# fal-ai-community/video-diffusion-speedrun

Hardware: AMD Instinct MI355X
Metric: train-step samples/sec (video latents) (higher is better)
Workload: dtype bf16; 1 GPU; C3b DiT-XL/2 bf16, latents [16,16,64,64] pt=2 -> 8192+16 tokens, ctx [512,4096]; per_gpu_batch=12, global_batch=12, parallelism=single, launch=eager, deterministic=False

## Files before the change

### video_diffusion_speedrun_amd/csrc/attention.hip

```cpp
#include "common.h"
#include <type_traits>
#include "prof.h"
#include "config.h"
#include "../../include/vds.h"
#include <cstdlib>

namespace {

constexpr float LOG2E = 1.4426950408889634f;
constexpr float LN2 = 0.6931471805599453f;

struct AttnP {
  int B, H, Lq, Lk, hd;
  const bf16_t* q; long q_sb, q_sh, q_sl;
  const bf16_t* k; long k_sb, k_sh, k_sl;
  const bf16_t* v; long v_sb, v_sh, v_sl;
  bf16_t* o; long o_sb, o_sh, o_sl;
  float* lse;
  const bf16_t* d_o; long do_sb, do_sh, do_sl;
  bf16_t* dq; long dq_sb, dq_sh, dq_sl;
  bf16_t* dk; long dk_sb, dk_sh, dk_sl;
  bf16_t* dv; long dv_sb, dv_sh, dv_sl;
  float* delta;
  float scale;
// ... 791 lines not shown
  DmaStage<64, HDP> dq_, dd_;
  dq_.init(p.q_sl, hd_q, wave, lane);
  dd_.init(p.do_sl, p.hd, wave, lane);
  const unsigned q_step = (unsigned)(64 * p.q_sl * 2), do_step = (unsigned)(64 * p.do_sl * 2);
  auto issue_tile = [&](int j, int par) {
    char* nb = qbuf + par * 2 * Q_TILE;
    dq_.issue(rq, nb, (unsigned)j * q_step, wave);
    dd_.issue(rdo, nb + Q_TILE, (unsigned)j * do_step, wave);
    if (wave == 0) {
      char* st = stats + par * 512;
      const unsigned sa = lds_addr_of(st);
      lds_dma4(rl2, sa, (unsigned)((j * 64 + lane) * 4));
      lds_dma4(rdl, sa + 256, (unsigned)((j * 64 + lane) * 4));
    }
  };
  const int nqt_all = (p.Lq + 63) / 64, jper = (nqt_all + p.q_split - 1) / (p.q_split > 0 ? p.q_split : 1);
  const int j0 = sp * jper, j1 = min(nqt_all, j0 + jper);
  issue_tile(j0, 0);

  bf16x8 kf[KSQ], vf[KSQ];
#pragma unroll
  for (int ks = 0; ks < KSQ; ++ks) {
    const int e = ks * 16 + 8 * h;
    unsigned offk = (unsigned)(((long)krow * p.k_sl + e) * 2);
    unsigned offv = (unsigned)(((long)krow * p.v_sl + e) * 2);
    if (e >= p.hd) { offk = 0xfffffff0u; offv = 0xfffffff0u; }
    kf[ks] = __builtin_bit_cast(bf16x8, __builtin_amdgcn_raw_buffer_load_b128(rk, offk, 0, 0));
    vf[ks] = __builtin_bit_cast(bf16x8, __builtin_amdgcn_raw_buffer_load_b128(rv, offv, 0, 0));
  }
  if constexpr (ONES) {
#pragma unroll
    for (int ks = 0; ks < KSQ; ++ks) kf[ks] = scale_frag(kf[ks], c);
    if (h == 1) {
      kf[KSQ - 1][0] = (__bf16)1.0f;
      kf[KSQ - 1][1] = (__bf16)1.0f;
    }
  }

  f32x16 dk[NDB], dv[NDB];
#pragma unroll
  for (int i = 0; i < NDB; ++i) { dk[i] = zero16(); dv[i] = zero16(); }
#pragma unroll
  for (int ks = 0; ks < KSQ; ++ks) { retire(kf[ks]); retire(vf[ks]); }
  VDS_WAIT_VM(0);
  __syncthreads();

  auto q_tile = [&](int j, auto PAR) {
    constexpr int par = decltype(PAR)::value;
    if (j + 1 < j1) issue_tile(j + 1, par ^ 1);
    const char* qt = qbuf + par * 2 * Q_TILE;
    const char* dot = qt + Q_TILE;
    const float* stl = reinterpret_cast<const float*>(stats + par * 512);
#pragma unroll
    for (int qb = 0; qb < 2; ++qb) {
      f32x16 s = zero16(), dp;
#pragma unroll
      for (int rg = 0; rg < 4; ++rg) {
        const f32x4 d4 = *reinterpret_cast<const f32x4*>(stl + 64 + qb * 32 + 8 * rg + 4 * h);
#pragma unroll
        for (int e = 0; e < 4; ++e) dp[4 * rg + e] = d4[e];
      }
      PRIO_HI();
#pragma unroll
      for (int ks = 0; ks < KSQ; ++ks) {
        s = mfma32(frag_row<HDP>(qt, qb * 32, ks, lane), kf[ks], s);
        dp = mfma32(frag_row<HDP>(dot, qb * 32, ks, lane), vf[ks], dp);
      }
      PRIO_LO();
      f32x16 pm;
      if constexpr (ONES) {
#pragma unroll
        for (int r = 0; r < 16; ++r) {
          const float pr = __builtin_amdgcn_exp2f(s[r]);
          pm[r] = pr;
          s[r] = pr * dp[r];
        }
      } else {
#pragma unroll
        for (int rg = 0; rg < 4; ++rg) {
          const f32x4 l4 = *reinterpret_cast<const f32x4*>(stl + qb * 32 + 8 * rg + 4 * h);
#pragma unroll
          for (int e = 0; e < 4; ++e) {
            const int r = 4 * rg + e;
            const float pr = __builtin_amdgcn_exp2f(s[r] * c - l4[e]);
            pm[r] = pr;
            s[r] = pr * dp[r];
          }
        }
      }
      PRIO_HI();
#pragma unroll
      for (int s2 = 0; s2 < 2; ++s2) {
        const bf16x8 pf = acc_frag(pm, s2);
        const bf16x8 df = acc_frag(s, s2);
#pragma unroll
        for (int db = 0; db < NDB; ++db) {
          dv[db] = mfma32(frag_tr<HDP>(dot, qb * 32 + 16 * s2, db * 32, lane), pf, dv[db]);
          dk[db] = mfma32(frag_tr<HDP>(qt, qb * 32 + 16 * s2, db * 32, lane), df, dk[db]);
        }
      }
      PRIO_LO();
    }
    VDS_WAIT_VM(0);
    __syncthreads();
  };
  for (int j = j0; j < j1; j += 2) {
    q_tile(j, std::integral_constant<int, 0>{});
    if (j + 1 < j1) q_tile(j + 1, std::integral_constant<int, 1>{});
  }
  if constexpr (KVLEN) {
    if (krow >= Lk) {
#pragma unroll
      for (int i = 0; i < NDB; ++i) { dk[i] = zero16(); dv[i] = zero16(); }
    }
  }
  if (krow < p.Lk) {
    if (p.q_split > 1) {
      float* part = p.dkv_part + ((((long)sp * p.B * p.H + bh) * p.Lk + krow) * 2) * p.hd;
      store_rows_f32<NDB>(part, dk, p.hd, h);
      store_rows_f32<NDB>(part + p.hd, dv, p.hd, h);
    } else {
      store_rows<NDB>(p.dk + b * p.dk_sb + hh * p.dk_sh + (long)krow * p.dk_sl, dk, p.scale, p.hd, h);
      store_rows<NDB>(p.dv + b * p.dv_sb + hh * p.dv_sh + (long)krow * p.dv_sl, dv, 1.0f, p.hd, h);
    }
  }
}

__device__ __forceinline__ f32x4 mfma16(bf16x8 a, bf16x8 b, f32x4 c) {
  return __builtin_amdgcn_mfma_f32_16x16x32_bf16(a, b, c, 0, 0, 0);
}
template <int HDP>
__device__ __forceinline__ bf16x8 frag16_row(const char* tile, int row0, int ks, int lane) {
  return *reinterpret_cast<const bf16x8*>(tile + imgb_off<HDP>(row0 + (lane & 15), ks * 4 + (lane >> 4)));
}
template <int HDP>
__device__ __forceinline__ bf16x8 frag16_tr(const char* tile, int r0, int d0, int lane) {
  const int g = lane >> 4, i = lane & 15, qq = i >> 2, pp = i & 3;
  const int row = r0 + 4 * g + qq;
  const int ch = (d0 >> 3) + (pp >> 1);
  const char* p0 = tile + imgb_off<HDP>(row, ch) + 8 * (pp & 1);
  const char* p1 = tile + imgb_off<HDP>(row + 16, ch) + 8 * (pp & 1);
  s16x4 lo = __builtin_amdgcn_ds_read_tr16_b64_v4i16((__attribute__((address_space(3))) s16x4*)LDS_PTR(p0));
  s16x4 hi = __builtin_amdgcn_ds_read_tr16_b64_v4i16((__attribute__((address_space(3))) s16x4*)LDS_PTR(p1));
  s16x8 r = {lo[0], lo[1], lo[2], lo[3], hi[0], hi[1], hi[2], hi[3]};
  return __builtin_bit_cast(bf16x8, r);
}
__device__ __forceinline__ bf16x8 pack2(const f32x4& a, const f32x4& b) {
  bf16x8 r;
#pragma unroll
  for (int j = 0; j < 4; ++j) { r[j] = (__bf16)a[j]; r[4 + j] = (__bf16)b[j]; }
  return r;
}

template <int HDP, bool QPAD = true, bool KVLEN = false>
__global__ __launch_bounds__(256, 2) void attn_bwd_dkv16_kernel(AttnP p) {
  static_assert(HDP == 96, "head_dim 72 layout (ones columns at 72, 73)");
  constexpr int KS = HDP / 32, NDB = 5, Q_TILE = 64 * HDP * 2;
  extern __shared__ __attribute__((aligned(16))) char smem[];
  char* qbuf = smem;
  char* stats = smem + 4 * Q_TILE;
  int bh, kt_idx;
  if (!decode_block(p.n_rt, p.tail_last, p.B * p.H, bh, kt_idx)) return;
  const int b = bh / p.H, hh = bh % p.H;
  const int tid = threadIdx.x, lane = tid & 63, g = lane >> 4;
  const int wave = __builtin_amdgcn_readfirstlane(tid >> 6);
  const int key0 = kt_idx * 128 + wave * 32;
  const int Lk = kv_len_of<KVLEN>(p, b);
  if constexpr (KVLEN) {
    if (kt_idx * 128 >= Lk) {
#pragma unroll
      for (int cb = 0; cb < 2; ++cb) {
        const int krow = key0 + cb * 16 + (lane & 15);
        store_zero_block(p.dk + b * p.dk_sb + hh * p.dk_sh + (long)krow * p.dk_sl, p.hd, g, krow < p.Lk, p.wide_dkv);
        store_zero_block(p.dv + b * p.dv_sb + hh * p.dv_sh + (long)krow * p.dv_sl, p.hd, g, krow < p.Lk, p.wide_dkv);
      }
      return;
    }
  }

  const int hd_q = QPAD ? p.hd + 8 : p.hd;
  const srd_t rq = slice_srd(p.q + b * p.q_sb + hh * p.q_sh, p.q_sl, p.Lq, hd_q);
  const srd_t rdo = slice_srd(p.d_o + b * p.do_sb + hh * p.do_sh, p.do_sl, p.Lq, p.hd);
  const __amdgpu_buffer_rsrc_t rk = slice_rsrc(p.k + b * p.k_sb + hh * p.k_sh, p.k_sl, Lk, p.hd);
  const __amdgpu_buffer_rsrc_t rv = slice_rsrc(p.v + b * p.v_sb + hh * p.v_sh, p.v_sl, Lk, p.hd);
  const long nrows = (long)p.B * p.H * p.Lq;
  const long srow0 = ((long)b * p.H + hh) * p.Lq;
  const srd_t rdl = make_srd(p.delta + srow0, (unsigned)(p.Lq * 4));
  const srd_t rl2 = make_srd(p.delta + nrows + srow0, (unsigned)(p.Lq * 4));
  const float c = p.scale * LOG2E;

  DmaStage<64, HDP, 1> dq_, dd_;
  dq_.init(p.q_sl, hd_q, wave, lane);
  dd_.init(p.do_sl, p.hd, wave, lane);
  const unsigned q_step = (unsigned)(64 * p.q_sl * 2), do_step = (unsigned)(64 * p.do_sl * 2);
  auto issue_tile = [&](int j, int par) {
    char* nb = qbuf + par * 2 * Q_TILE;
    dq_.issue(rq, nb, (unsigned)j * q_step, wave);
    dd_.issue(rdo, nb + Q_TILE, (unsigned)j * do_step, wave);
    if (wave == 0) {
      char* st = stats + par * 512;
      const unsigned sa = lds_addr_of(st);
      lds_dma4(rl2, sa, (unsigned)((j * 64 + lane) * 4));
      lds_dma4(rdl, sa + 256, (unsigned)((j * 64 + lane) * 4));
    }
  };
  issue_tile(0, 0);

  bf16x8 kf[2][KS], vf[2][KS];
#pragma unroll
  for (int cb = 0; cb < 2; ++cb) {
    const int krow = key0 + cb * 16 + (lane & 15);
#pragma unroll
    for (int ks = 0; ks < KS; ++ks) {
      const int e = ks * 32 + 8 * g;
      unsigned offk = (unsigned)(((long)krow * p.k_sl + e) * 2);
      unsigned offv = (unsigned)(((long)krow * p.v_sl + e) * 2);
      if (e >= p.hd) { offk = 0xfffffff0u; offv = 0xfffffff0u; }
      kf[cb][ks] = __builtin_bit_cast(bf16x8, __builtin_amdgcn_raw_buffer_load_b128(rk, offk, 0, 0));
      vf[cb][ks] = __builtin_bit_cast(bf16x8, __builtin_amdgcn_raw_buffer_load_b128(rv, offv, 0, 0));
    }
  }
#pragma unroll
  for (int cb = 0; cb < 2; ++cb) {
#pragma unroll
    for (int ks = 0; ks < KS; ++ks) { kf[cb][ks] = scale_frag(kf[cb][ks], c); retire(vf[cb][ks]); }
    if (g == 1) {
      kf[cb][KS - 1][0] = (__bf16)1.0f;
      kf[cb][KS - 1][1] = (__bf16)1.0f;
    }
  }

  f32x4 dk[NDB][2], dv[NDB][2];
#pragma unroll
  for (int i = 0; i < NDB; ++i)
#pragma unroll
    for (int cb = 0; cb < 2; ++cb) { dk[i][cb] = f32x4{0.f, 0.f, 0.f, 0.f}; dv[i][cb] = f32x4{0.f, 0.f, 0.f, 0.f}; }
  const int nqt = (p.Lq + 63) / 64;
  VDS_WAIT_VM(0);
  __syncthreads();

  auto q_tile = [&](int j, auto PAR, auto NKBT) {
    constexpr int par = decltype(PAR)::value;
    constexpr int NKB = decltype(NKBT)::value;
    if (j + 1 < nqt) issue_tile(j + 1, par ^ 1);
    const char* qt = qbuf + par * 2 * Q_TILE;
    const char* dot = qt + Q_TILE;
    const float* stl = reinterpret_cast<const float*>(stats + par * 512);
    if constexpr (NKB > 0)
#pragma unroll
    for (int qb = 0; qb < 2; ++qb) {
      f32x4 s[2][2], dp[2][2];
#pragma unroll
      for (int rb = 0; rb < 2; ++rb) {
        const f32x4 d4 = *reinterpret_cast<const f32x4*>(stl + 64 + qb * 32 + rb * 16 + 4 * g);
        f32x4 s0 = f32x4{0.f, 0.f, 0.f, 0.f};
        if constexpr (!QPAD) s0 = -*reinterpret_cast<const f32x4*>(stl + qb * 32 + rb * 16 + 4 * g);
#pragma unroll
        for (int cb = 0; cb < NKB; ++cb) { s[rb][cb] = s0; dp[rb][cb] = d4; }
      }
      PRIO_HI();
#pragma unroll
      for (int ks = 0; ks < KS; ++ks)
#pragma unroll
        for (int rb = 0; rb < 2; ++rb) {
          const bf16x8 aq = frag16_row<HDP>(qt, qb * 32 + rb * 16, ks, lane);
          const bf16x8 ad = frag16_row<HDP>(dot, qb * 32 + rb * 16, ks, lane);
#pragma unroll
          for (int cb = 0; cb < NKB; ++cb) {
            s[rb][cb] = mfma16(aq, kf[cb][ks], s[rb][cb]);
            dp[rb][cb] = mfma16(ad, vf[cb][ks], dp[rb][cb]);
          }
        }
      PRIO_LO();
#pragma unroll
      for (int rb = 0; rb < 2; ++rb)
#pragma unroll
        for (int cb = 0; cb < NKB; ++cb)
#pragma unroll
          for (int r = 0; r < 4; ++r) s[rb][cb][r] = __builtin_amdgcn_exp2f(s[rb][cb][r]);
#pragma unroll
      for (int rb = 0; rb < 2; ++rb)
#pragma unroll
        for (int cb = 0; cb < NKB; ++cb)
#pragma unroll
          for (int r = 0; r < 4; ++r) dp[rb][cb][r] *= s[rb][cb][r];
      bf16x8 pf[2], df[2];
#pragma unroll
      for (int cb = 0; cb < NKB; ++cb) {
        pf[cb] = pack2(s[0][cb], s[1][cb]);
        df[cb] = pack2(dp[0][cb], dp[1][cb]);
      }
      PRIO_HI();
#pragma unroll
      for (int db = 0; db < NDB; ++db) {
        const bf16x8 ado = frag16_tr<HDP>(dot, qb * 32, db * 16, lane);
        const bf16x8 aqt = frag16_tr<HDP>(qt, qb * 32, db * 16, lane);
#pragma unroll
        for (int cb = 0; cb < NKB; ++cb) {
          dv[db][cb] = mfma16(ado, pf[cb], dv[db][cb]);
          dk[db][cb] = mfma16(aqt, df[cb], dk[db][cb]);
        }
      }
      PRIO_LO();
    }
    VDS_WAIT_VM(0);
    __syncthreads();
  };
  auto run = [&](auto NKBT) {
    for (int j = 0; j < nqt; j += 2) {
      q_tile(j, std::integral_constant<int, 0>{}, NKBT);
      if (j + 1 < nqt) q_tile(j + 1, std::integral_constant<int, 1>{}, NKBT);
    }
  };
  const int nkb = min(2, max(0, (Lk - key0 + 15) >> 4));
  if (nkb == 2) run(std::integral_constant<int, 2>{});
  else if (nkb == 1) run(std::integral_constant<int, 1>{});
  else run(std::integral_constant<int, 0>{});
#pragma unroll
  for (int cb = 0; cb < 2; ++cb) {
    const int krow = key0 + cb * 16 + (lane & 15);
    float vk[NDB][4], vv[NDB][4];
#pragma unroll
    for (int db = 0; db < NDB; ++db)
#pragma unroll
      for (int e = 0; e < 4; ++e) { vk[db][e] = dk[db][cb][e]; vv[db][e] = dv[db][cb][e]; }
    if constexpr (KVLEN) {
      if (krow >= Lk) {
#pragma unroll
        for (int db = 0; db < NDB; ++db)
#pragma unroll
          for (int e = 0; e < 4; ++e) { vk[db][e] = 0.f; vv[db][e] = 0.f; }
      }
    }
    store_block_bf16_t(vk, p.scale, p.dk + b * p.dk_sb + hh * p.dk_sh + (long)krow * p.dk_sl, p.hd, g, krow < p.Lk, p.wide_dkv);
    store_block_bf16_t(vv, 1.0f, p.dv + b * p.dv_sb + hh * p.dv_sh + (long)krow * p.dv_sl, p.hd, g, krow < p.Lk, p.wide_dkv);
  }
}

__device__ __forceinline__ float max3f(float a, float b, float c) { return __builtin_fmaxf(__builtin_fmaxf(a, b), c); }
__device__ __forceinline__ float max_over_lane_groups(float x) {
  auto a = __builtin_amdgcn_permlane16_swap(__float_as_uint(x), __float_as_uint(x), false, false);
  x = fmaxf(__uint_as_float(a[0]), __uint_as_float(a[1]));
  auto b = __builtin_amdgcn_permlane32_swap(__float_as_uint(x), __float_as_uint(x), false, false);
  return fmaxf(__uint_as_float(b[0]), __uint_as_float(b[1]));
}

template <int HDP, bool KVLEN = false>
__global__ __launch_bounds__(256, 2) void attn_fwd16_kernel(AttnP p) {
  static_assert(HDP == 96, "head_dim 72 layout (ones columns at 72, 73 / 72, 76)");
  constexpr int KS = HDP / 32, NDB = 5, TILE = 64 * HDP * 2;
  extern __shared__ __attribute__((aligned(16))) char smem[];
  int bh, qt;
  if (!decode_block(p.n_rt, p.tail_last, p.B * p.H, bh, qt)) return;
  const int b = bh / p.H, hh = bh % p.H;
  const int tid = threadIdx.x, lane = tid & 63, g = lane >> 4;
  const int wave = __builtin_amdgcn_readfirstlane(tid >> 6);
  const int qrow0 = qt * 256 + wave * 64 + (lane & 15);
  const int hd_kv = p.hd + 8;
  const int Lk = kv_len_of<KVLEN>(p, b);
  if constexpr (KVLEN) {
    if (Lk == 0) {
#pragma unroll
      for (int cb = 0; cb < 4; ++cb) {
        const int qrow = qrow0 + 16 * cb;
        store_zero_block(p.o + b * p.o_sb + hh * p.o_sh + (long)qrow * p.o_sl, p.hd, g, qrow < p.Lq, p.wide_o);
        if (qrow < p.Lq && g == 0) p.lse[((long)b * p.H + hh) * p.Lq + qrow] = 0.0f;
      }
      return;
    }
  }

  const __amdgpu_buffer_rsrc_t rq = slice_rsrc(p.q + b * p.q_sb + hh * p.q_sh, p.q_sl, p.Lq, p.hd);
  const srd_t rk = slice_srd(p.k + b * p.k_sb + hh * p.k_sh, p.k_sl, Lk, hd_kv);
  const srd_t rv = slice_srd(p.v + b * p.v_sb + hh * p.v_sh, p.v_sl, Lk, hd_kv);
  DmaStage<64, HDP, 1> dk, dv;
  dk.init(p.k_sl, hd_kv, wave, lane);
  dv.init(p.v_sl, hd_kv, wave, lane);
  const unsigned k_step = (unsigned)(64 * p.k_sl * 2), v_step = (unsigned)(64 * p.v_sl * 2);
  dk.issue(rk, smem, 0, wave);
  dv.issue(rv, smem + TILE, 0, wave);

  const float c = p.scale * LOG2E;
  bf16x8 qf[4][KS];
#pragma unroll
  for (int cb = 0; cb < 4; ++cb)
#pragma unroll
    for (int ks = 0; ks < KS; ++ks) {
      const int e = ks * 32 + 8 * g;
      unsigned off = (unsigned)(((long)(qrow0 + 16 * cb) * p.q_sl + e) * 2);
      if (e >= p.hd) off = 0xfffffff0u;
      qf[cb][ks] = __builtin_bit_cast(bf16x8, __builtin_amdgcn_raw_buffer_load_b128(rq, off, 0, 0));
    }
#pragma unroll
  for (int cb = 0; cb < 4; ++cb)
#pragma unroll
    for (int ks = 0; ks < KS; ++ks) qf[cb][ks] = scale_frag(qf[cb][ks], c);

  f32x4 o[NDB][4];
#pragma unroll
  for (int db = 0; db < NDB; ++db)
#pragma unroll
    for (int cb = 0; cb < 4; ++cb) o[db][cb] = f32x4{0.f, 0.f, 0.f, 0.f};
  float m[4] = {0.f, 0.f, 0.f, 0.f};
  const int nkt = (Lk + 63) / 64;
  VDS_WAIT_VM(0);
  __syncthreads();

  auto kv_tile = [&](int j, auto PAR, auto NCBT) {
    constexpr int par = decltype(PAR)::value;
    constexpr int NCB = decltype(NCBT)::value;
    if (j + 1 < nkt) {
      char* nk = smem + (par ^ 1) * 2 * TILE;
      dk.issue(rk, nk, (unsigned)(j + 1) * k_step, wave);
      dv.issue(rv, nk + TILE, (unsigned)(j + 1) * v_step, wave);
    }
    const char* kt = smem + par * 2 * TILE;
    const char* vt = kt + TILE;
    if constexpr (NCB > 0)
#pragma unroll
    for (int kb = 0; kb < 2; ++kb) {
      f32x4 s[2][4];
#pragma unroll
      for (int rb = 0; rb < 2; ++rb)
#pragma unroll
        for (int cb = 0; cb < NCB; ++cb) s[rb][cb] = f32x4{0.f, 0.f, 0.f, 0.f};
      PRIO_HI();
#pragma unroll
      for (int ks = 0; ks < KS; ++ks)
#pragma unroll
        for (int rb = 0; rb < 2; ++rb) {
          const bf16x8 ak = frag16_row<HDP>(kt, kb * 32 + rb * 16, ks, lane);
#pragma unroll
          for (int cb = 0; cb < NCB; ++cb) s[rb][cb] = mfma16(ak, qf[cb][ks], s[rb][cb]);
        }
      PRIO_LO();
      const bool first = (j == 0) && (kb == 0);
      float mx[4];
#pragma unroll
      for (int cb = 0; cb < NCB; ++cb) {
        mx[cb] = max3f(max3f(s[0][cb][0], s[0][cb][1], s[0][cb][2]), max3f(s[0][cb][3], s[1][cb][0], s[1][cb][1]),
                       fmaxf(s[1][cb][2], s[1][cb][3]));
      }
      float mxa = mx[0];
      if constexpr (NCB == 4) mxa = fmaxf(max3f(mx[0], mx[1], mx[2]), mx[3]);
      else {
#pragma unroll
        for (int cb = 1; cb < NCB; ++cb) mxa = fmaxf(mxa, mx[cb]);
      }
      if (first || __builtin_amdgcn_ballot_w64(mxa > LAZY_THR) != 0) {
        asm volatile("; rescale" ::: "memory");
#pragma unroll
        for (int cb = 0; cb < NCB; ++cb) {
          const float mxf = max_over_lane_groups(mx[cb]);
          const float m_new = bf2f(f2bf(m[cb] + (first ? mxf : fmaxf(mxf, 0.f))));
          const float delta = m_new - m[cb];
          const float alpha = first ? 1.0f : __builtin_amdgcn_exp2f(-delta);
          m[cb] = m_new;
#pragma unroll
          for (int db = 0; db < NDB; ++db) o[db][cb] *= alpha;
#pragma unroll
          for (int rb = 0; rb < 2; ++rb)
#pragma unroll
            for (int r = 0; r < 4; ++r) s[rb][cb][r] -= delta;
          if (g == 1) qf[cb][KS - 1][0] = (__bf16)(-m_new);
        }
      }
      bf16x8 pf[4];
#pragma unroll
      for (int cb = 0; cb < NCB; ++cb) {
#pragma unroll
// ... 175 lines not shown
#pragma unroll
          for (int r = 0; r < 4; ++r) s[rb][cb][r] = __builtin_amdgcn_exp2f(s[rb][cb][r]);
#pragma unroll
      for (int rb = 0; rb < 2; ++rb)
#pragma unroll
        for (int cb = 0; cb < NCB; ++cb)
#pragma unroll
          for (int r = 0; r < 4; ++r) s[rb][cb][r] *= dp[rb][cb][r];
      bf16x8 df[NQ];
#pragma unroll
      for (int cb = 0; cb < NCB; ++cb) df[cb] = pack2(s[0][cb], s[1][cb]);
#pragma unroll
      for (int db = 0; db < NDB; ++db) {
        const bf16x8 akt = frag16_tr<HDP>(kt, kb * 32, db * 16, lane);
#pragma unroll
        for (int cb = 0; cb < NCB; ++cb) dq[db][cb] = mfma16(akt, df[cb], dq[db][cb]);
      }
    }
    VDS_WAIT_VM(0);
    __syncthreads();
  };
  auto run = [&](auto NCBT) {
    for (int j = 0; j < nkt; j += 2) {
      kv_tile(j, std::integral_constant<int, 0>{}, NCBT);
      if (j + 1 < nkt) kv_tile(j + 1, std::integral_constant<int, 1>{}, NCBT);
    }
  };
  const int ncb = min(NQ, max(0, (p.Lq - (qt * (64 * NQ) + wave * (16 * NQ)) + 15) >> 4));
  if (ncb == NQ) run(std::integral_constant<int, NQ>{});
  else if (ncb == 2) run(std::integral_constant<int, 2>{});
  else if (ncb == 1) run(std::integral_constant<int, 1>{});
  else run(std::integral_constant<int, 0>{});
#pragma unroll
  for (int cb = 0; cb < NQ; ++cb) {
    const int qrow = qrow0 + 16 * cb;
    float vq[NDB][4];
#pragma unroll
    for (int db = 0; db < NDB; ++db)
#pragma unroll
      for (int e = 0; e < 4; ++e) vq[db][e] = dq[db][cb][e];
    store_block_bf16_t(vq, p.scale, p.dq + b * p.dq_sb + hh * p.dq_sh + (long)qrow * p.dq_sl, p.hd, g, qrow < p.Lq, p.wide_dq);
  }
}

bool rows16(const void* base, long sb, long sh, long sl) {
  return base && ((uintptr_t)base % 16 == 0) && (sb % 8 == 0) && (sh % 8 == 0) && (sl % 8 == 0);
}

AttnP to_p(const vds_attn_args* a) {
  AttnP p;
  p.B = a->B; p.H = a->H; p.Lq = a->Lq; p.Lk = a->Lk; p.hd = a->head_dim;
  p.q = (const bf16_t*)a->q; p.q_sb = a->q_sb; p.q_sh = a->q_sh; p.q_sl = a->q_sl;
  p.k = (const bf16_t*)a->k; p.k_sb = a->k_sb; p.k_sh = a->k_sh; p.k_sl = a->k_sl;
  p.v = (const bf16_t*)a->v; p.v_sb = a->v_sb; p.v_sh = a->v_sh; p.v_sl = a->v_sl;
  p.o = (bf16_t*)a->o; p.o_sb = a->o_sb; p.o_sh = a->o_sh; p.o_sl = a->o_sl;
  p.lse = a->lse;
  p.d_o = (const bf16_t*)a->d_o; p.do_sb = a->do_sb; p.do_sh = a->do_sh; p.do_sl = a->do_sl;
  p.dq = (bf16_t*)a->dq; p.dq_sb = a->dq_sb; p.dq_sh = a->dq_sh; p.dq_sl = a->dq_sl;
  p.dk = (bf16_t*)a->dk; p.dk_sb = a->dk_sb; p.dk_sh = a->dk_sh; p.dk_sl = a->dk_sl;
  p.dv = (bf16_t*)a->dv; p.dv_sb = a->dv_sb; p.dv_sh = a->dv_sh; p.dv_sl = a->dv_sl;
  p.delta = a->delta;
  p.scale = 1.0f / sqrtf((float)a->head_dim);
  p.n_rt = 0;
  p.tail_last = 0;
  p.kv_pad_ones = a->kv_pad_ones;
  p.q_split = 1;
  p.dkv_part = nullptr;
  p.kv_lens = nullptr;
  const bool wide_on = vdscfg::geti(vdscfg::ATTN_WIDE_STORES) != 0;
  p.wide_o = wide_on && p.hd > 64 && rows16(p.o, p.o_sb, p.o_sh, p.o_sl);
  p.wide_dq = wide_on && p.hd > 64 && rows16(p.dq, p.dq_sb, p.dq_sh, p.dq_sl);
  p.wide_dkv = wide_on && p.hd > 64 && rows16(p.dk, p.dk_sb, p.dk_sh, p.dk_sl) && rows16(p.dv, p.dv_sb, p.dv_sh, p.dv_sl);
  return p;
}

int kernel_instance(int hd) {
  if (hd <= 0 || (hd & 7) || hd > 128) return 0;
  return hd <= 32 ? 32 : hd <= 64 ? 64 : hd <= 80 ? 80 : hd <= 96 ? 96 : 128;
}

bool strides_ok(const vds_attn_args* a, bool bwd) {
  auto ok = [](int64_t s) { return (s & 7) == 0; };
  bool r = ok(a->q_sb) && ok(a->q_sh) && ok(a->q_sl) && ok(a->k_sb) && ok(a->k_sh) && ok(a->k_sl) &&
           ok(a->v_sb) && ok(a->v_sh) && ok(a->v_sl) && (a->o_sb % 4 == 0) && (a->o_sh % 4 == 0) && (a->o_sl % 4 == 0);
  if (bwd)
    r = r && ok(a->do_sb) && ok(a->do_sh) && ok(a->do_sl) && (a->dq_sl % 4 == 0) && (a->dk_sl % 4 == 0) &&
        (a->dv_sl % 4 == 0) && (a->dq_sh % 4 == 0) && (a->dk_sh % 4 == 0) && (a->dv_sh % 4 == 0) &&
        (a->dq_sb % 4 == 0) && (a->dk_sb % 4 == 0) && (a->dv_sb % 4 == 0);
  return r;
}

constexpr int ATTN_VARIANT_DEFAULT = 7;
int attn_variant() { return vdscfg::geti(vdscfg::ATTN_MFMA16) & 7; }

template <typename K>
void set_lds(K kern, int bytes) {
  (void)hipFuncSetAttribute(reinterpret_cast<const void*>(kern), hipFuncAttributeMaxDynamicSharedMemorySize, bytes);
}

static int tail_last_for(int L, int tile) {
  return (vdscfg::geti(vdscfg::ATTN_TAIL_LAST) && L > tile && (L % tile) != 0) ? 1 : 0;
}

template <int HDP, int HDQ, bool KVLEN = false>
int run_fwd(AttnP p, hipStream_t s) {
  constexpr int LDS = 4 * 64 * HDP * 2;
  static bool once = false;
  if (!once) {
    set_lds(attn_fwd_kernel<HDP, HDQ, 2, true, KVLEN>, LDS);
    if constexpr (HDP <= 96) set_lds(attn_fwd_wide_kernel<HDP, HDQ, false, KVLEN>, LDS);
    if constexpr (HDP == 96 && HDQ == 80) set_lds(attn_fwd_wide_kernel<HDP, HDQ, true, KVLEN>, LDS);
    if constexpr (HDP == 96 && HDQ == 80) set_lds(attn_fwd16_kernel<HDP, KVLEN>, LDS);
    once = true;
  }
  const int wide = vdscfg::geti(vdscfg::ATTN_FWD_WIDE);
  bool use_wide = false;
  if constexpr (HDP == 96) use_wide = wide == 1 || (wide == 2 && p.Lq >= 2048);
  if constexpr (HDP == 64) use_wide = wide == 1 || (wide == 2 && p.Lq >= 2048);
  p.n_rt = cdiv(p.Lq, use_wide ? 256 : 128);
  p.tail_last = tail_last_for(p.Lq, use_wide ? 256 : 128);
  const int grid = cdiv(p.B * p.H, 8) * 8 * p.n_rt;
  const double fl = 4.0 * p.B * p.H * (double)p.Lq * p.Lk * p.hd;
  const bool ones_fwd = HDP == 96 && HDQ == 80 && use_wide && p.kv_pad_ones && p.hd == 72;
  vdsprof::Scope ps(ones_fwd && p.kv_pad_ones == 1 ? VDS_PROF_ATTN_FWD : VDS_PROF_ATTN_FWD_PLAIN, s, fl,
                    2.0 * p.B * p.H * p.hd * (2.0 * p.Lq + 2.0 * p.Lk));
  if constexpr (HDP == 64) {
    if (use_wide) {
      hipLaunchKernelGGL((attn_fwd_wide_kernel<HDP, HDQ, false, KVLEN>), dim3(grid), dim3(256), LDS, s, p);
      return hipGetLastError() == hipSuccess ? VDS_OK : VDS_ERR_LAUNCH;
    }
  }
  if constexpr (HDP == 96) {
    if (use_wide) {
      bool done = false;
      if constexpr (HDQ == 80) {
        if (p.kv_pad_ones && p.hd == 72) {
          if (attn_variant() & 4) hipLaunchKernelGGL((attn_fwd16_kernel<HDP, KVLEN>), dim3(grid), dim3(256), LDS, s, p);
          else hipLaunchKernelGGL((attn_fwd_wide_kernel<HDP, HDQ, true, KVLEN>), dim3(grid), dim3(256), LDS, s, p);
          done = true;
        }
      }
      if (!done) hipLaunchKernelGGL((attn_fwd_wide_kernel<HDP, HDQ, false, KVLEN>), dim3(grid), dim3(256), LDS, s, p);
      return hipGetLastError() == hipSuccess ? VDS_OK : VDS_ERR_LAUNCH;
    }
  }
  hipLaunchKernelGGL((attn_fwd_kernel<HDP, HDQ, 2, true, KVLEN>), dim3(grid), dim3(256), LDS, s, p);
  return hipGetLastError() == hipSuccess ? VDS_OK : VDS_ERR_LAUNCH;
}

int dkv_qsplit(int B, int H, int Lq, int Lk) {
  const long wgs = (long)cdiv(B * H, 8) * 8 * cdiv(Lk, 128);
  const int nqt = cdiv(Lq, 64);
  if (wgs >= 3 * 512 || nqt < 16) return 1;
  long sp = (3 * 512 + wgs - 1) / wgs;
  if (sp > nqt / 8) sp = nqt / 8;
  return (int)(sp < 1 ? 1 : sp > 16 ? 16 : sp);
}

template <int HDP, int HDQ, bool KVLEN = false>
int run_bwd(AttnP p, hipStream_t s, size_t ws_floats) {
  constexpr int LDS_DQ = 4 * 64 * HDP * 2;
  constexpr int LDS_DKV = 4 * 64 * HDP * 2 + 2 * 128 * 4;
  static bool once = false;
  if (!once) {
    set_lds(attn_bwd_dq_kernel<HDP, HDQ, false, KVLEN>, LDS_DQ);
    if constexpr (HDP == 96 && HDQ == 80) set_lds(attn_bwd_dq_kernel<HDP, HDQ, true, KVLEN>, LDS_DQ);
    set_lds(attn_bwd_dkv_kernel<HDP, HDQ, false, KVLEN>, LDS_DKV);
    if constexpr (HDP == 96 && HDQ == 80) set_lds(attn_bwd_dkv_kernel<HDP, HDQ, true>, LDS_DKV);
    if constexpr (HDP == 96 && HDQ == 80) set_lds(attn_bwd_dkv16_kernel<HDP>, LDS_DKV);
    if constexpr (HDP == 96 && HDQ == 80) set_lds(attn_bwd_dkv16_kernel<HDP, false, KVLEN>, LDS_DKV);
    if constexpr (HDP == 96 && HDQ == 80) set_lds(attn_bwd_dq16_kernel<HDP, false, KVLEN>, LDS_DQ);
    if constexpr (HDP == 96 && HDQ == 80) set_lds(attn_bwd_dq16_kernel<HDP, true, KVLEN>, LDS_DQ);
    once = true;
  }
  const long rows = (long)p.B * p.H * p.Lq;
  const double prod = 2.0 * p.B * p.H * (double)p.Lq * p.Lk * p.hd;
  const double qb = 2.0 * p.B * p.H * p.hd * (double)p.Lq, kb = 2.0 * p.B * p.H * p.hd * (double)p.Lk;
  bool fold = false;
  if constexpr (HDP == 96 && HDQ == 80) fold = p.kv_pad_ones && p.hd == 72 && (attn_variant() & 2) && vdscfg::geti(vdscfg::ATTN_DELTA_FOLD);
  auto launch_dq = [&]() {
    p.n_rt = cdiv(p.Lq, 128);
    p.tail_last = tail_last_for(p.Lq, 128);
    const int grid = cdiv(p.B * p.H, 8) * 8 * p.n_rt;
    bool ones = false;
    if constexpr (HDP == 96 && HDQ == 80) ones = p.kv_pad_ones && p.hd == 72;
    vdsprof::Scope ps(ones && p.kv_pad_ones == 1 ? VDS_PROF_ATTN_BWD_DQ : VDS_PROF_ATTN_BWD_DQ_PLAIN, s, 2.0 * prod,
                      (fold ? 4.0 : 3.0) * qb + 2.0 * kb);
    if constexpr (HDP == 96 && HDQ == 80) {
      if (fold)
        hipLaunchKernelGGL((attn_bwd_dq16_kernel<HDP, true, KVLEN>), dim3(grid), dim3(256), LDS_DQ, s, p);
      else if (ones && (attn_variant() & 2))
        hipLaunchKernelGGL((attn_bwd_dq16_kernel<HDP, false, KVLEN>), dim3(grid), dim3(256), LDS_DQ, s, p);
      else if (ones)
        hipLaunchKernelGGL((attn_bwd_dq_kernel<HDP, HDQ, true, KVLEN>), dim3(grid), dim3(256), LDS_DQ, s, p);
    }
    if (!ones) hipLaunchKernelGGL((attn_bwd_dq_kernel<HDP, HDQ, false, KVLEN>), dim3(grid), dim3(256), LDS_DQ, s, p);
  };
  if (fold) launch_dq();
  else {
    vdsprof::Scope ps(VDS_PROF_ATTN_BWD_DELTA, s, 2.0 * rows * p.hd, 2.0 * qb);
    const bool tokmajor = p.o_sh == p.hd && p.do_sh == p.hd && p.o_sl == (long)p.H * p.hd && p.do_sl == p.o_sl &&
                          (p.o_sl & 7) == 0 && (p.o_sb & 7) == 0 && (p.do_sb & 7) == 0 && p.H * p.hd <= 1536 && p.H <= 64;
    if (tokmajor)
      hipLaunchKernelGGL(attn_delta_tokmajor_kernel, dim3((unsigned)(((long)p.B * p.Lq + 3) / 4)), dim3(256), 0, s, p);
    else
      hipLaunchKernelGGL(attn_delta_kernel, dim3((unsigned)((rows + 3) / 4)), dim3(256), 0, s, p);
  }
  p.n_rt = cdiv(p.Lk, 128);
  p.tail_last = tail_last_for(p.Lk, 128);
  int grid = cdiv(p.B * p.H, 8) * 8 * p.n_rt;
  {
    bool ones_kv = false;
    if constexpr (HDP == 96 && HDQ == 80) ones_kv = p.kv_pad_ones == 1 && p.hd == 72;
    vdsprof::Scope ps(ones_kv ? VDS_PROF_ATTN_BWD_DKV : VDS_PROF_ATTN_BWD_DKV_PLAIN, s, 2.0 * prod, 2.0 * qb + 4.0 * kb);
    if constexpr (HDP == 96 && HDQ == 80) {
      if (ones_kv && (attn_variant() & 1))
        hipLaunchKernelGGL((attn_bwd_dkv16_kernel<HDP>), dim3(grid), dim3(256), LDS_DKV, s, p);
      else if (ones_kv)
        hipLaunchKernelGGL((attn_bwd_dkv_kernel<HDP, HDQ, true>), dim3(grid), dim3(256), LDS_DKV, s, p);
    }
    bool done16 = false;
    if constexpr (HDP == 96 && HDQ == 80) {
      const int x16 = vdscfg::geti(vdscfg::CROSS_DKV16);
      if (!ones_kv && p.kv_pad_ones == 2 && p.hd == 72 && x16 && ((long)grid >= 512 || x16 == 2) && (attn_variant() & 1)) {
        hipLaunchKernelGGL((attn_bwd_dkv16_kernel<HDP, false, KVLEN>), dim3(grid), dim3(256), LDS_DKV, s, p);
        done16 = true;
      }
    }
    if (!ones_kv && !done16) {
      const int force = vdscfg::geti(vdscfg::ATTN_QSPLIT);
      const int split = force > 0 ? force : dkv_qsplit(p.B, p.H, p.Lq, p.Lk);
      const size_t need = (size_t)2 * rows + (size_t)split * p.B * p.H * p.Lk * 2 * p.hd;
      if (split > 1 && (p.hd & 3) == 0 && ws_floats >= need && (p.dk_sl & 3) == 0) {
        p.q_split = split;
        p.dkv_part = p.delta + 2 * rows;
        p.tail_last = 0;
        const int g2 = cdiv(p.B * p.H, 8) * 8 * p.n_rt * split;
        hipLaunchKernelGGL((attn_bwd_dkv_kernel<HDP, HDQ, false, KVLEN>), dim3(g2), dim3(256), LDS_DKV, s, p);
        const long n = (long)p.B * p.H * p.Lk * 2 * (p.hd >> 2);
        hipLaunchKernelGGL(dkv_reduce_kernel<KVLEN>, dim3((unsigned)((n + 255) / 256)), dim3(256), 0, s, p);
        p.q_split = 1;
        p.dkv_part = nullptr;
      } else {
        hipLaunchKernelGGL((attn_bwd_dkv_kernel<HDP, HDQ, false, KVLEN>), dim3(grid), dim3(256), LDS_DKV, s, p);
      }
    }
  }
  if (!fold) launch_dq();
  return hipGetLastError() == hipSuccess ? VDS_OK : VDS_ERR_LAUNCH;
}

}

__global__ __launch_bounds__(256) void kv_pad_ones_kernel(const bf16_t* kv, long ld, int kcol0, int vcol0, bf16_t* kp,
                                                          bf16_t* vp, int B, int Lk, int H, int hd, int hdp) {
  const int cpr = hdp >> 3;
  const long n = (long)B * H * Lk * cpr;
  const long gid = (long)blockIdx.x * 256 + threadIdx.x;
  if (gid >= n) return;
  const int which = blockIdx.y;
  const int c = (int)(gid % cpr);
  const long row = gid / cpr;
  const int l = (int)(row % Lk);
  const int h = (int)((row / Lk) % H);
  const int b = (int)(row / ((long)Lk * H));
  u32x4 w = {0u, 0u, 0u, 0u};
  if (c * 8 < hd) {
    w = *reinterpret_cast<const u32x4*>(kv + ((long)b * Lk + l) * ld + (which ? vcol0 : kcol0) + h * hd + c * 8);
  } else if (c * 8 == hd) {
    w[0] = which ? 0x00003f80u : 0x3f803f80u;
    w[2] = which ? 0x00003f80u : 0u;
  }
  *reinterpret_cast<u32x4*>((which ? vp : kp) + row * hdp + c * 8) = w;
}

extern "C" int vds_kv_pad_ones(const void* kv, int64_t ld, int32_t k_col0, int32_t v_col0, void* kp, void* vp, int32_t B,
                               int32_t Lk, int32_t H, int32_t hd, int32_t hdp, vds_stream_t stream) {
  if (!kv || !kp || !vp || B <= 0 || Lk <= 0 || H <= 0 || hd <= 0) return VDS_ERR_ARG;
  if ((hd & 7) || (hdp & 7) || hdp < hd + 8 || (ld & 7) || (k_col0 & 7) || (v_col0 & 7)) return VDS_ERR_ARG;
  const long n = (long)B * H * Lk * (hdp >> 3);
  hipLaunchKernelGGL(kv_pad_ones_kernel, dim3((unsigned)((n + 255) / 256), 2), dim3(256), 0, (hipStream_t)stream,
                     (const bf16_t*)kv, (long)ld, k_col0, v_col0, (bf16_t*)kp, (bf16_t*)vp, B, Lk, H, hd, hdp);
  return hipGetLastError() == hipSuccess ? VDS_OK : VDS_ERR_LAUNCH;
}

extern "C" int vds_attn_set_variant(int32_t mask) {
  const int prev = attn_variant();
  if (mask < -1 || mask > 7) return VDS_ERR_ARG;
  vdscfg::g_val[vdscfg::ATTN_MFMA16] = mask < 0 ? ATTN_VARIANT_DEFAULT : mask;
  return prev;
}

extern "C" int vds_attn_fwd(const vds_attn_args* a, vds_stream_t stream) {
  if (!a || !a->q || !a->k || !a->v || !a->o || !a->lse || a->Lq <= 0 || a->Lk <= 0) return VDS_ERR_ARG;
  if (!strides_ok(a, false)) return VDS_ERR_ARG;
  AttnP p = to_p(a);
  hipStream_t s = (hipStream_t)stream;
  switch (kernel_instance(a->head_dim)) {
    case 32: return run_fwd<32, 32>(p, s);
    case 64: return run_fwd<64, 64>(p, s);
    case 80: return run_fwd<96, 80>(p, s);
    case 96: return run_fwd<96, 96>(p, s);
    case 128: return run_fwd<128, 128>(p, s);
    default: return VDS_ERR_UNSUPPORTED;
  }
}

extern "C" int vds_attn_fwd_kvlen(const vds_attn_args* a, const int32_t* kv_lens, vds_stream_t stream) {
  if (!a) return VDS_ERR_ARG;
  if (!kv_lens) return vds_attn_fwd(a, stream);
  if (a->kv_pad_ones == 1) return VDS_ERR_ARG;
  if (!a->q || !a->k || !a->v || !a->o || !a->lse || a->Lq <= 0 || a->Lk <= 0) return VDS_ERR_ARG;
  if (!strides_ok(a, false)) return VDS_ERR_ARG;
  AttnP p = to_p(a);
  p.kv_lens = kv_lens;
  hipStream_t s = (hipStream_t)stream;
  switch (kernel_instance(a->head_dim)) {
    case 32: return run_fwd<32, 32, true>(p, s);
    case 64: return run_fwd<64, 64, true>(p, s);
    case 80: return run_fwd<96, 80, true>(p, s);
    case 96: return run_fwd<96, 96, true>(p, s);
    case 128: return run_fwd<128, 128, true>(p, s);
    default: return VDS_ERR_UNSUPPORTED;
  }
}

extern "C" size_t vds_attn_bwd_workspace_bytes(const vds_attn_args* a) {
  if (!a || a->B <= 0 || a->H <= 0 || a->Lq <= 0) return 0;
  size_t fl = (size_t)2 * a->B * a->H * a->Lq;
  if (a->Lk > 0 && a->head_dim > 0 && a->kv_pad_ones != 1)
    fl += (size_t)dkv_qsplit(a->B, a->H, a->Lq, a->Lk) * a->B * a->H * a->Lk * 2 * a->head_dim;
  return fl * sizeof(float);
}

extern "C" int vds_attn_bwd(const vds_attn_args* a, vds_stream_t stream) {
  if (!a || !a->q || !a->k || !a->v || !a->o || !a->lse || !a->d_o || !a->dq || !a->dk || !a->dv || !a->delta)
    return VDS_ERR_ARG;
  if (!strides_ok(a, true)) return VDS_ERR_ARG;
  AttnP p = to_p(a);
  hipStream_t s = (hipStream_t)stream;
  const size_t ws = a->ws_floats > 0 ? (size_t)a->ws_floats : (size_t)2 * a->B * a->H * a->Lq;
  switch (kernel_instance(a->head_dim)) {
    case 32: return run_bwd<32, 32>(p, s, ws);
    case 64: return run_bwd<64, 64>(p, s, ws);
    case 80: return run_bwd<96, 80>(p, s, ws);
    case 96: return run_bwd<96, 96>(p, s, ws);
    case 128: return run_bwd<128, 128>(p, s, ws);
    default: return VDS_ERR_UNSUPPORTED;
  }
}

extern "C" int vds_attn_bwd_kvlen(const vds_attn_args* a, const int32_t* kv_lens, vds_stream_t stream) {
  if (!a) return VDS_ERR_ARG;
  if (!kv_lens) return vds_attn_bwd(a, stream);
  if (a->kv_pad_ones == 1) return VDS_ERR_ARG;
  if (!a->q || !a->k || !a->v || !a->o || !a->lse || !a->d_o || !a->dq || !a->dk || !a->dv || !a->delta || a->Lq <= 0 ||
      a->Lk <= 0)
    return VDS_ERR_ARG;
  if (!strides_ok(a, true)) return VDS_ERR_ARG;
  AttnP p = to_p(a);
  p.kv_lens = kv_lens;
  hipStream_t s = (hipStream_t)stream;
  const size_t ws = a->ws_floats > 0 ? (size_t)a->ws_floats : (size_t)2 * a->B * a->H * a->Lq;
  switch (kernel_instance(a->head_dim)) {
    case 32: return run_bwd<32, 32, true>(p, s, ws);
    case 64: return run_bwd<64, 64, true>(p, s, ws);
    case 80: return run_bwd<96, 80, true>(p, s, ws);
    case 96: return run_bwd<96, 96, true>(p, s, ws);
    case 128: return run_bwd<128, 128, true>(p, s, ws);
    default: return VDS_ERR_UNSUPPORTED;
  }
}
```

Baseline: 14.84 samples/s.

## Add query-split variant to dkv16 cross-attention backward kernel

```diff
diff --git a/video_diffusion_speedrun_amd/csrc/attention.hip b/video_diffusion_speedrun_amd/csrc/attention.hip
--- a/video_diffusion_speedrun_amd/csrc/attention.hip
+++ b/video_diffusion_speedrun_amd/csrc/attention.hip
@@ -967,15 +967,23 @@
   return r;
 }
 
-template <int HDP, bool QPAD = true, bool KVLEN = false>
+template <int HDP, bool QPAD = true, bool KVLEN = false, bool QSPLIT = false>
 __global__ __launch_bounds__(256, 2) void attn_bwd_dkv16_kernel(AttnP p) {
   static_assert(HDP == 96, "head_dim 72 layout (ones columns at 72, 73)");
   constexpr int KS = HDP / 32, NDB = 5, Q_TILE = 64 * HDP * 2;
   extern __shared__ __attribute__((aligned(16))) char smem[];
   char* qbuf = smem;
   char* stats = smem + 4 * Q_TILE;
-  int bh, kt_idx;
-  if (!decode_block(p.n_rt, p.tail_last, p.B * p.H, bh, kt_idx)) return;
+  int bh, kt_idx, sp = 0;
+  if constexpr (QSPLIT) {
+    const int per = p.n_rt * p.q_split, pid = blockIdx.x, idx = pid >> 3;
+    bh = (idx / per) * 8 + (pid & 7);
+    if (bh >= p.B * p.H) return;
+    kt_idx = (idx % per) % p.n_rt;
+    sp = (idx % per) / p.n_rt;
+  } else {
+    if (!decode_block(p.n_rt, p.tail_last, p.B * p.H, bh, kt_idx)) return;
+  }
   const int b = bh / p.H, hh = bh % p.H;
   const int tid = threadIdx.x, lane = tid & 63, g = lane >> 4;
   const int wave = __builtin_amdgcn_readfirstlane(tid >> 6);
@@ -983,6 +991,7 @@
   const int Lk = kv_len_of<KVLEN>(p, b);
   if constexpr (KVLEN) {
     if (kt_idx * 128 >= Lk) {
+      if constexpr (QSPLIT) return;
 #pragma unroll
       for (int cb = 0; cb < 2; ++cb) {
         const int krow = key0 + cb * 16 + (lane & 15);
@@ -1019,7 +1028,15 @@
       lds_dma4(rdl, sa + 256, (unsigned)((j * 64 + lane) * 4));
     }
   };
-  issue_tile(0, 0);
+  int js0 = 0, js1 = 0;
+  if constexpr (QSPLIT) {
+    const int n = (p.Lq + 63) / 64;
+    js0 = (int)((long)sp * n / p.q_split);
+    js1 = (int)((long)(sp + 1) * n / p.q_split);
+    if (js0 < js1) issue_tile(js0, 0);
+  } else {
+    issue_tile(0, 0);
+  }
 
   bf16x8 kf[2][KS], vf[2][KS];
 #pragma unroll
@@ -1057,7 +1074,7 @@
   auto q_tile = [&](int j, auto PAR, auto NKBT) {
     constexpr int par = decltype(PAR)::value;
     constexpr int NKB = decltype(NKBT)::value;
-    if (j + 1 < nqt) issue_tile(j + 1, par ^ 1);
+    if (j + 1 < (QSPLIT ? js1 : nqt)) issue_tile(j + 1, par ^ 1);
     const char* qt = qbuf + par * 2 * Q_TILE;
     const char* dot = qt + Q_TILE;
     const float* stl = reinterpret_cast<const float*>(stats + par * 512);
@@ -1122,15 +1139,33 @@
     __syncthreads();
   };
   auto run = [&](auto NKBT) {
-    for (int j = 0; j < nqt; j += 2) {
+    for (int j = (QSPLIT ? js0 : 0); j < (QSPLIT ? js1 : nqt); j += 2) {
       q_tile(j, std::integral_constant<int, 0>{}, NKBT);
-      if (j + 1 < nqt) q_tile(j + 1, std::integral_constant<int, 1>{}, NKBT);
+      if (j + 1 < (QSPLIT ? js1 : nqt)) q_tile(j + 1, std::integral_constant<int, 1>{}, NKBT);
     }
   };
   const int nkb = min(2, max(0, (Lk - key0 + 15) >> 4));
   if (nkb == 2) run(std::integral_constant<int, 2>{});
   else if (nkb == 1) run(std::integral_constant<int, 1>{});
   else run(std::integral_constant<int, 0>{});
+  if constexpr (QSPLIT) {
+#pragma unroll
+    for (int cb = 0; cb < 2; ++cb) {
+      const int krow = key0 + cb * 16 + (lane & 15);
+      if (krow < Lk) {
+        float* part = p.dkv_part + ((((long)sp * p.B * p.H + bh) * p.Lk + krow) * 2) * p.hd;
+#pragma unroll
+        for (int db = 0; db < NDB; ++db) {
+          const int d = db * 16 + 4 * g;
+          if (d < p.hd) {
+            *reinterpret_cast<f32x4*>(part + d) = dk[db][cb];
+            *reinterpret_cast<f32x4*>(part + p.hd + d) = dv[db][cb];
+          }
+        }
+      }
+    }
+    return;
+  }
 #pragma unroll
   for (int cb = 0; cb < 2; ++cb) {
     const int krow = key0 + cb * 16 + (lane & 15);
@@ -1612,9 +1647,11 @@
   const long wgs = (long)cdiv(B * H, 8) * 8 * cdiv(Lk, 128);
   const int nqt = cdiv(Lq, 64);
   if (wgs >= 3 * 512 || nqt < 16) return 1;
-  long sp = (3 * 512 + wgs - 1) / wgs;
-  if (sp > nqt / 8) sp = nqt / 8;
-  return (int)(sp < 1 ? 1 : sp > 16 ? 16 : sp);
+  const long cap = nqt / 8 < 16 ? nqt / 8 : 16;
+  for (long sp = 1; sp <= cap; ++sp)
+    if ((wgs * sp) % 512 == 0) return (int)sp;
+  const long sp = (3 * 512 + wgs - 1) / wgs;
+  return (int)(sp > cap ? cap : sp);
 }
 
 template <int HDP, int HDQ, bool KVLEN = false>
@@ -1629,6 +1666,7 @@
     if constexpr (HDP == 96 && HDQ == 80) set_lds(attn_bwd_dkv_kernel<HDP, HDQ, true>, LDS_DKV);
     if constexpr (HDP == 96 && HDQ == 80) set_lds(attn_bwd_dkv16_kernel<HDP>, LDS_DKV);
     if constexpr (HDP == 96 && HDQ == 80) set_lds(attn_bwd_dkv16_kernel<HDP, false, KVLEN>, LDS_DKV);
+    if constexpr (HDP == 96 && HDQ == 80) set_lds(attn_bwd_dkv16_kernel<HDP, false, KVLEN, true>, LDS_DKV);
     if constexpr (HDP == 96 && HDQ == 80) set_lds(attn_bwd_dq16_kernel<HDP, false, KVLEN>, LDS_DQ);
     if constexpr (HDP == 96 && HDQ == 80) set_lds(attn_bwd_dq16_kernel<HDP, true, KVLEN>, LDS_DQ);
     once = true;
@@ -1679,31 +1717,37 @@
       else if (ones_kv)
         hipLaunchKernelGGL((attn_bwd_dkv_kernel<HDP, HDQ, true>), dim3(grid), dim3(256), LDS_DKV, s, p);
     }
+    const int force = vdscfg::geti(vdscfg::ATTN_QSPLIT);
+    const int split = force > 0 ? force : dkv_qsplit(p.B, p.H, p.Lq, p.Lk);
+    const size_t need = (size_t)2 * rows + (size_t)split * p.B * p.H * p.Lk * 2 * p.hd;
+    const bool can_split = !ones_kv && split > 1 && (p.hd & 3) == 0 && ws_floats >= need && (p.dk_sl & 3) == 0;
+    auto launch_split = [&](auto kern) {
+      p.q_split = split;
+      p.dkv_part = p.delta + 2 * rows;
+      p.tail_last = 0;
+      const int g2 = cdiv(p.B * p.H, 8) * 8 * p.n_rt * split;
+      hipLaunchKernelGGL(kern, dim3(g2), dim3(256), LDS_DKV, s, p);
+      const long n = (long)p.B * p.H * p.Lk * 2 * (p.hd >> 2);
+      hipLaunchKernelGGL(dkv_reduce_kernel<KVLEN>, dim3((unsigned)((n + 255) / 256)), dim3(256), 0, s, p);
+      p.q_split = 1;
+      p.dkv_part = nullptr;
+    };
     bool done16 = false;
     if constexpr (HDP == 96 && HDQ == 80) {
       const int x16 = vdscfg::geti(vdscfg::CROSS_DKV16);
-      if (!ones_kv && p.kv_pad_ones == 2 && p.hd == 72 && x16 && ((long)grid >= 512 || x16 == 2) && (attn_variant() & 1)) {
-        hipLaunchKernelGGL((attn_bwd_dkv16_kernel<HDP, false, KVLEN>), dim3(grid), dim3(256), LDS_DKV, s, p);
-        done16 = true;
+      if (!ones_kv && p.kv_pad_ones == 2 && p.hd == 72 && x16 && (attn_variant() & 1)) {
+        if (can_split) {
+          launch_split(attn_bwd_dkv16_kernel<HDP, false, KVLEN, true>);
+          done16 = true;
+        } else if ((long)grid >= 512 || x16 == 2) {
+          hipLaunchKernelGGL((attn_bwd_dkv16_kernel<HDP, false, KVLEN>), dim3(grid), dim3(256), LDS_DKV, s, p);
+          done16 = true;
+        }
       }
     }
     if (!ones_kv && !done16) {
-      const int force = vdscfg::geti(vdscfg::ATTN_QSPLIT);
-      const int split = force > 0 ? force : dkv_qsplit(p.B, p.H, p.Lq, p.Lk);
-      const size_t need = (size_t)2 * rows + (size_t)split * p.B * p.H * p.Lk * 2 * p.hd;
-      if (split > 1 && (p.hd & 3) == 0 && ws_floats >= need && (p.dk_sl & 3) == 0) {
-        p.q_split = split;
-        p.dkv_part = p.delta + 2 * rows;
-        p.tail_last = 0;
-        const int g2 = cdiv(p.B * p.H, 8) * 8 * p.n_rt * split;
-        hipLaunchKernelGGL((attn_bwd_dkv_kernel<HDP, HDQ, false, KVLEN>), dim3(g2), dim3(256), LDS_DKV, s, p);
-        const long n = (long)p.B * p.H * p.Lk * 2 * (p.hd >> 2);
-        hipLaunchKernelGGL(dkv_reduce_kernel<KVLEN>, dim3((unsigned)((n + 255) / 256)), dim3(256), 0, s, p);
-        p.q_split = 1;
-        p.dkv_part = nullptr;
-      } else {
-        hipLaunchKernelGGL((attn_bwd_dkv_kernel<HDP, HDQ, false, KVLEN>), dim3(grid), dim3(256), LDS_DKV, s, p);
-      }
+      if (can_split) launch_split(attn_bwd_dkv_kernel<HDP, HDQ, false, KVLEN>);
+      else hipLaunchKernelGGL((attn_bwd_dkv_kernel<HDP, HDQ, false, KVLEN>), dim3(grid), dim3(256), LDS_DKV, s, p);
     }
   }
   if (!fold) launch_dq();
```

Result: no change. 14.80 samples/s (-0.2%).
